# timspilak/cloud_merger

Hardware: AMD Instinct MI355X
Metric: merged+voxelized points/sec at 5 cm leaf, 4×1 M-pt inputs; HBM GB/s fraction (higher is better)
Workload: dtype f32

## Files before the change

### cloud_merger_amd/csrc/cm_common.hpp

```cpp
#pragma once
#include <hip/hip_runtime.h>
#include <stddef.h>
#include <stdint.h>

#include "cm_device.h"

namespace {

struct Pt { float x, y, z, i; };

#if defined(__HIP_DEVICE_COMPILE__)
#define CM_GLOBAL_AS __attribute__((address_space(1)))
#else
#define CM_GLOBAL_AS
#endif
typedef const CM_GLOBAL_AS unsigned char* cm_gptr;
typedef float cm_v4f __attribute__((ext_vector_type(4)));

__device__ __forceinline__ float load_f32_unaligned(cm_gptr p) {
    float f;
    __builtin_memcpy(&f, (const void*)p, 4);
    return f;
}

// ... 347 lines not shown
    if (!overflow && d[0] * d[1] * d[2] > 2147483647LL) overflow = true;
    if (overflow) { g.status = CM_DEV_OVERFLOW; return; }
    unsigned long long cells = 1;
#pragma unroll
    for (int a = 0; a < 3; ++a) {
        const int lo = static_cast<int>(floorf(__fmul_rn(g.min_p[a], inv[a])));
        const int hi = static_cast<int>(floorf(__fmul_rn(g.max_p[a], inv[a])));
        g.min_b[a] = lo; g.max_b[a] = hi; g.div_b[a] = hi - lo + 1;
        cells *= static_cast<unsigned long long>(hi - lo + 1);
    }
    if (cells > 0xFFFFFFFFull) { g.status = CM_DEV_OVERFLOW; return; }
    uint32_t bits = 1;
    while (bits < 32 && (cells - 1) >> bits) ++bits;
    g.key_bits = bits;
    g.n_passes = (bits + CM_RADIX_BITS - 1) / CM_RADIX_BITS;
}

struct BoxGrid {
    float inv0, inv1, inv2, fb0, fb1, fb2;
    uint32_t d0, d1, d2;
    uint32_t mul1, mul2l, mul2h;
};

__device__ __forceinline__ BoxGrid box_grid_of(const CmFrameDev* __restrict__ fd, int use_cell = 0) {
    BoxGrid b;
    const int32_t* min_b = use_cell ? fd->cell_min_b : fd->box_min_b;
    const int32_t* div_b = use_cell ? fd->cell_div_b : fd->box_div_b;
    const float* inv = use_cell ? fd->inv_cell : fd->inv_leaf;
    b.inv0 = inv[0]; b.inv1 = inv[1]; b.inv2 = inv[2];
    b.fb0 = static_cast<float>(min_b[0]); b.fb1 = static_cast<float>(min_b[1]); b.fb2 = static_cast<float>(min_b[2]);
    b.d0 = static_cast<uint32_t>(div_b[0]); b.d1 = static_cast<uint32_t>(div_b[1]); b.d2 = static_cast<uint32_t>(div_b[2]);
    b.mul1 = b.d0;
    const uint32_t mul2 = b.d0 * b.d1;
    b.mul2l = mul2 & 0xFFFu; b.mul2h = mul2 >> 12;
    return b;
}

__device__ __forceinline__ uint32_t box_index(const BoxGrid& b, uint32_t c0, uint32_t c1, uint32_t c2) {
    uint32_t hi = __umul24(c2, b.mul2h);
    asm("" : "+v"(hi));
    return c0 + __umul24(c1, b.mul1) + __umul24(c2, b.mul2l) + (hi << 12);
}

__device__ __forceinline__ uint32_t key_of(const BoxGrid& b, float x, float y, float z, bool* inside) {
    const uint32_t c0 = static_cast<uint32_t>(static_cast<int>(__fsub_rn(floorf(__fmul_rn(x, b.inv0)), b.fb0)));
    const uint32_t c1 = static_cast<uint32_t>(static_cast<int>(__fsub_rn(floorf(__fmul_rn(y, b.inv1)), b.fb1)));
    const uint32_t c2 = static_cast<uint32_t>(static_cast<int>(__fsub_rn(floorf(__fmul_rn(z, b.inv2)), b.fb2)));
// ... 237 lines not shown
```

### cloud_merger_amd/csrc/cm_kernels.h

```cpp
#pragma once
#include <hip/hip_runtime.h>
#include <stdint.h>

#include "cm_device.h"

void cmk_setup(hipStream_t s, const CmFrameDev& f, CmFrameDev* d_frame, CmTileDev* d_tiles);
void cmk_minmax(hipStream_t s, const CmFrameDev* fd, float* partials, uint32_t n_blocks, const unsigned char* mask);
void cmk_keys(hipStream_t s, const CmFrameDev* fd, CmFrameState* st, uint32_t* keys, uint32_t* hist,
              uint32_t* grp_acc, uint32_t* grp_clear_a, uint32_t* grp_clear_b, uint32_t n_group_words,
              uint32_t n_clear_a_words, uint32_t* seg_groups, uint32_t n_seg_groups, const float* partials,
              uint32_t n_partials, int from_crop, int use_cell, const unsigned char* mask,
              const CmFrameState* st_outlier, uint32_t n_tiles);
void cmk_outlier_mask(hipStream_t s, const CmFrameDev* fd, const CmFrameState* st, const uint32_t* keys_a,
                      const uint32_t* vals_a, const uint32_t* keys_b, const uint32_t* vals_b, void* sorted_pts,
                      void* rows, unsigned char* mask, uint32_t n_padded, const unsigned char* cls, uint32_t* pend_n,
                      bool already_gathered = false);
void cmk_sorted_rows(hipStream_t s, const CmFrameDev* fd, const CmFrameState* st, const uint32_t* keys_a, const uint32_t* vals_a,
                     const uint32_t* keys_b, const uint32_t* vals_b, void* sorted_pts, void* rows, uint32_t n_padded,
                     bool already_gathered);
void cmk_hist(hipStream_t s, const CmFrameState* st, const uint32_t* keys, uint32_t* hist, uint32_t* grp,
              uint32_t pass, uint32_t n_tiles);
void cmk_gscan(hipStream_t s, const CmFrameState* st, uint32_t* grp, uint32_t* totals, uint32_t pass,
               uint32_t n_groups);
void cmk_scatter(hipStream_t s, CmFrameState* st, const uint32_t* keys_in, const uint32_t* vals_in,
// ... 18 lines not shown
void cmk_merged(hipStream_t s, const CmFrameDev* fd, uint32_t* tile_counts, uint32_t* total, void* out,
                uint32_t n_tiles, const unsigned char* mask);

void cmk2_hist0(hipStream_t s, const CmFrameDev& f, CmFrameDev* fd, CmTileDev* tiles, bool do_setup, CmFrameState* st, uint32_t* hist, uint32_t* grp_acc,
                uint32_t* grp_clear_a, uint32_t* grp_clear_b, uint32_t n_group_words, uint32_t n_clear_a_words,
                unsigned long long* tile_state, uint32_t n_tile_state, float* records, int grid_mode, int check_box,
                uint32_t shift0, uint32_t n_global_passes, uint32_t n_tiles, const unsigned char* mask,
                const CmFrameState* st_outlier, int use_cell = 0, void* compact_out = nullptr, uint32_t* wave_cnt = nullptr);
void cmk2_hist(hipStream_t s, const CmFrameState* st, const unsigned char* dig, uint32_t* hist, uint32_t* grp,
               uint32_t n_tiles);
void cmk2_scatter(hipStream_t s, bool first, const CmFrameDev* fd, const CmTileDev* tiles, CmFrameState* st, const void* rec_in, void* rec_out,
                  unsigned char* dig_out, const uint32_t* hist, const uint32_t* grp, const uint32_t* totals,
                  uint32_t shift, uint32_t next_shift, uint32_t n_tiles, uint32_t n_groups, uint32_t n_padded,
                  const float* records, uint32_t n_records, int fold, const unsigned char* mask, int use_cell = 0,
                  const void* compact_in = nullptr, const uint32_t* wave_cnt = nullptr, int debug_swap = 0,
                  uint32_t* tile_kept = nullptr, bool sparse = false,
                  bool ballot = false);
void cmk2_local(hipStream_t s, const CmFrameDev* fd, CmFrameState* st, CmFrameState* st_next, uint32_t* host_state,
                const void* rec, unsigned long long* tile_state, uint32_t* ticket, void* out, uint32_t* out_key,
                uint32_t* out_cnt, void* partial_out, uint32_t low_bits, uint32_t n_padded);
void cmk2_local_sort(hipStream_t s, const CmFrameDev* fd, CmFrameState* st, uint32_t* host_state, const void* rec,
                     uint32_t* keys_sorted, void* recs_sorted, uint32_t low_bits, uint32_t n_padded);

void cmk3_local(hipStream_t s, const CmFrameDev* fd, CmFrameState* st, uint32_t* host_state, const void* rec, void* tile_info,
                uint32_t* grp_cnt, void* stage, uint32_t* stage_key, uint32_t* stage_cnt, bool partial, uint32_t low_bits,
                uint32_t n_slots,
                const uint32_t* spl = nullptr, const uint32_t* bofs = nullptr, uint32_t n_buckets = 0, uint32_t* spl_next = nullptr,
                bool ballot = false,
                uint32_t sub_shift = 0,
                const unsigned char* dig = nullptr);
void cmk3_local_big(hipStream_t s, const CmFrameDev* fd, CmFrameState* st, uint32_t* host_state, const void* rec, void* tile_info,
                    uint32_t* grp_cnt, void* stage, uint32_t* stage_key, uint32_t* stage_cnt, const uint32_t* spl, const uint32_t* bofs,
                    uint32_t n_buckets, uint32_t* spl_next, const uint32_t* big_list, bool ballot);
void cmk3_compact(hipStream_t s, const CmFrameState* st, CmFrameState* st_next, uint32_t* host_state, const void* tile_info,
                  const uint32_t* grp_cnt, const void* stage, const uint32_t* stage_key, const uint32_t* stage_cnt, void* out,
                  uint32_t* out_key, uint32_t* out_cnt, bool partial, uint32_t n_padded, uint32_t n_buckets = 0);

void cmk4_hist(hipStream_t s, const CmFrameDev& f, CmFrameDev* fd, CmTileDev* tiles, bool do_setup, CmFrameState* st,
               const uint32_t* spl, uint32_t* cnt, uint16_t* bid, unsigned long long* tile_state, uint32_t n_tile_state, float* records,
               int grid_mode, int check_box, uint32_t n_tiles,
               uint32_t n_buckets,
               uint32_t* big_list,
               uint32_t sub_shift,
               uint32_t* resident);
void cmk4_colscan(hipStream_t s, CmFrameState* st, uint32_t* host_state, uint32_t* cnt, uint32_t* totals, uint32_t n_tiles,
                  uint32_t cap, uint32_t cap_big, uint32_t* big_list);
void cmk4_scatter(hipStream_t s, const CmFrameDev* fd, const CmTileDev* tiles, CmFrameState* st, const uint16_t* bid,
                  const uint32_t* cnt, const uint32_t* totals, uint32_t* bofs, uint32_t n_buckets, void* rec_out,
                  const float* records, uint32_t n_records, int fold, uint32_t* tile_kept, uint32_t n_tiles,
                  unsigned char* dig_out,
                  bool ballot = false, const uint32_t* big_list = nullptr,
                  uint32_t sub_shift = 0);

void cmkg_setup(hipStream_t s, const CmGroundDev& g, CmGroundDev* d_ground);
// ... 59 lines not shown
```

### cloud_merger_amd/csrc/cm_kernels_v3.hip

```cpp
#include <hip/hip_runtime.h>
#include <stddef.h>
#include <stdint.h>

#include "cm_common.hpp"
#include "cm_device.h"
#include "cm_kernels.h"

namespace {

__device__ __forceinline__ float wave_sum_f32_fixed(float v) {
#define CM3_FADD(ctrl, rmask) v = __fadd_rn(v, __int_as_float(__builtin_amdgcn_update_dpp(0, __float_as_int(v), ctrl, rmask, 0xf, false)))
    CM3_FADD(0x111, 0xf); CM3_FADD(0x112, 0xf); CM3_FADD(0x114, 0xf); CM3_FADD(0x118, 0xf);
    CM3_FADD(0x142, 0xa); CM3_FADD(0x143, 0xc);
#undef CM3_FADD
    return __int_as_float(__builtin_amdgcn_readlane(__float_as_int(v), 63));
}

#define SCAL(x) static_cast<uint32_t>(__builtin_amdgcn_readfirstlane(static_cast<int>(x)))

struct Job3 {
    uint32_t p, key, kid, cnt;
    float sx, sy, sz, sw;
};
#define CM3_EXT_SEQ 16u
#define CM3_RUN_MAX (1u << 20)

CM_PHASE_DECLARE(g_phase_k3);

template <int LT, int LCAP, int LBLOCK, int WPS, bool PARTIAL, bool QUANT, bool BALLOT, bool SUB>
__global__ __launch_bounds__(LBLOCK, WPS) void k3_local(const CmFrameDev* __restrict__ fd,
                                                      CmFrameState* __restrict__ st,
                                                      uint32_t* __restrict__ host_state,
                                                      const float4* __restrict__ rec,
                                                      uint2* __restrict__ tile_info,
                                                      uint32_t* __restrict__ grp_cnt,
                                                      float4* __restrict__ stage,
                                                      uint32_t* __restrict__ stage_key,
                                                      uint32_t* __restrict__ stage_cnt,
                                                      uint32_t low_bits,
                                                      const uint32_t* __restrict__ spl, const uint32_t* __restrict__ bofs,
                                                      uint32_t n_buckets, uint32_t* __restrict__ spl_next,
                                                      const uint32_t* __restrict__ big_list, uint32_t sub_shift,
                                                      const unsigned char* __restrict__ dig) {
    constexpr int LWAVES = LBLOCK / 64, LITEMS = (LCAP + LBLOCK - 1) / LBLOCK, EXT0 = LBLOCK < 256 ? LBLOCK : 256;
    constexpr int WB = SUB ? 9 : 10, BINS = 1 << WB, HWORDS = BINS / 2;
    constexpr uint32_t MAXJ = LWAVES * HWORDS * 4 / sizeof(Job3);
    static_assert(LT == 4 * LBLOCK && LCAP <= 0x7FFE && HWORDS <= LBLOCK && LWAVES * HWORDS * 2 >= LCAP, "tile geometry");
    __shared__ uint32_t sk[LCAP];
    __shared__ uint16_t si[LCAP];
    __shared__ uint32_t whist[LWAVES][HWORDS];
    __shared__ uint32_t lds[2 * LWAVES];
    __shared__ uint32_t s_a, s_keyprev, s_bad, s_njobs;
    __shared__ uint16_t sp[SUB ? LCAP : 1];
    static_assert(!SUB || QUANT, "shared bins are a variant of the quantile finish");
    Job3* jobs = reinterpret_cast<Job3*>(&whist[0][0]);

    if (QUANT && big_list && blockIdx.x >= big_list[0]) return;
    PH_START();
    const int lane = threadIdx.x & 63;
    const uint32_t w = SCAL(threadIdx.x >> 6);
    if (st->status != CM_DEV_OK || st->outside) return;
    if (QUANT && st->quant_abort) return;
    const uint32_t n = SCAL(st->n_valid);
    const uint32_t n_lt = QUANT ? n_buckets : (n + LT - 1) / LT;
    uint32_t tile_ = blockIdx.x;
    if (SUB) {
        const uint32_t x = blockIdx.x & 7u, j = blockIdx.x >> 3;
        tile_ = (((((j >> sub_shift) << 3) + x) << sub_shift) + (j & ((1u << sub_shift) - 1u)));
    }
    if (QUANT && big_list) {
        if (tile_ >= SCAL(big_list[0])) return;
        tile_ = SCAL(big_list[1 + tile_]);
    }
    const uint32_t tile = tile_;
    if (tile >= n_lt) return;
    const BoxGrid b = box_grid_of(fd);
    const uint32_t L = QUANT ? 1u : low_bits;
    const uint32_t min_pts = SCAL((!PARTIAL && fd->min_pts > 1) ? fd->min_pts : 1u);

    const uint32_t bin = SUB ? tile >> sub_shift : tile;
    uint32_t base = QUANT ? SCAL(bofs[bin]) : tile * LT;
    const uint32_t rbase = base;
    const uint32_t q_end = QUANT ? SCAL(bofs[bin + 1]) : 0u;
    bool q_big = QUANT && !SUB && (q_end - base) > static_cast<uint32_t>(LCAP);
    if (QUANT && q_big && !big_list && (q_end - base) <= CM4_CAP_BIG) return;
    uint32_t nom = QUANT ? (q_big ? 0u : q_end - base) : min(static_cast<uint32_t>(LT), n - base);
    const uint32_t key_end = QUANT ? (fd->box_key_bits < 32u ? (1u << fd->box_key_bits) : 0xFFFFFFFFu) : 0u;
    const uint32_t q_lo = QUANT ? SCAL(spl[tile]) : 0u;
    const uint32_t q_hi = QUANT ? min(SCAL(spl[tile + 1]), key_end) : 0u;
    bool q_bad = false;
    if (SUB) {
        const uint32_t sub = tile & ((1u << sub_shift) - 1u);
        uint32_t kept = 0, below_t = 0;
        for (uint32_t off = rbase & ~15u; off < q_end; off += 16 * LBLOCK) {
            const uint32_t p0 = off + 16 * threadIdx.x;
            uint4 d = make_uint4(0xFFFFFFFFu, 0xFFFFFFFFu, 0xFFFFFFFFu, 0xFFFFFFFFu);
            if (p0 < q_end) d = *reinterpret_cast<const uint4*>(dig + p0);
            const uint32_t dw[4] = {d.x, d.y, d.z, d.w};
            uint32_t mm = 0;
#pragma unroll
            for (int i = 0; i < 16; ++i) {
                const uint32_t p = p0 + i, v = (dw[i >> 2] >> (8 * (i & 3))) & 0xFFu;
                const bool valid = p >= rbase && p < q_end;
                mm |= (valid && v == sub) ? (1u << i) : 0u;
                below_t += (valid && v < sub) ? 1u : 0u;
            }
            uint32_t tot;
            uint32_t pos = kept + block_excl_scan<LWAVES>(static_cast<uint32_t>(__builtin_popcount(mm)), lds, &tot);
            while (mm) {
                const uint32_t i = static_cast<uint32_t>(__builtin_ctz(mm));
                mm &= mm - 1u;
                if (pos < static_cast<uint32_t>(LCAP)) sp[pos] = static_cast<uint16_t>(p0 + i - rbase);
                ++pos;
            }
            kept += SCAL(tot);
        }
        uint32_t below;
        (void)block_excl_scan<LWAVES>(below_t, lds, &below);
        base = rbase + SCAL(below);
        q_big = kept > static_cast<uint32_t>(LCAP);
        nom = q_big ? 0u : kept;
        __syncthreads();
    }
    if (QUANT) {
        constexpr int HALF = LITEMS / 2;
#pragma unroll
        for (int h = 0; h < 2; ++h) {
            if (h == 1 && nom <= static_cast<uint32_t>(HALF * LBLOCK)) break;
            float4 r4[HALF];
#pragma unroll
            for (int r = 0; r < HALF; ++r) {
                const uint32_t q = (h * HALF + r) * LBLOCK + threadIdx.x;
                r4[r] = (q < nom) ? rec[rbase + (SUB ? sp[q < nom ? q : 0u] : q)] : make_float4(0.f, 0.f, 0.f, 0.f);
            }
#pragma unroll
            for (int r = 0; r < HALF; ++r) {
                const uint32_t q = (h * HALF + r) * LBLOCK + threadIdx.x;
                if (q < nom) {
                    const uint32_t k = key_of(b, r4[r]);
                    sk[q] = k;
                    q_bad = q_bad || k < q_lo || k >= q_hi;
                }
            }
        }
        if (threadIdx.x == 0) { s_keyprev = 0u; s_a = 0u; s_bad = 0u; s_njobs = 0u; }
    } else {
        float4 r4[4];
#pragma unroll
        for (int r = 0; r < 4; ++r) {
            const uint32_t q = r * LBLOCK + threadIdx.x;
            r4[r] = (q < nom) ? rec[base + q] : make_float4(0.f, 0.f, 0.f, 0.f);
        }
        const uint32_t j0 = base + LT + threadIdx.x;
        const bool has_e = threadIdx.x < EXT0 && nom == LT && j0 < n;
        const float4 e4 = has_e ? rec[j0] : make_float4(0.f, 0.f, 0.f, 0.f);
        float4 pv = make_float4(0.f, 0.f, 0.f, 0.f);
        if (threadIdx.x == 0 && base > 0) pv = rec[base - 1];
#pragma unroll
        for (int r = 0; r < 4; ++r) {
            const uint32_t q = r * LBLOCK + threadIdx.x;
            if (q < nom) sk[q] = key_of(b, r4[r]);
        }
        if (has_e) sk[LT + threadIdx.x] = key_of(b, e4);
        if (threadIdx.x == 0) { s_keyprev = base > 0 ? key_of(b, pv) : 0u; s_a = 0xFFFFFFFFu; s_bad = 0u; s_njobs = 0u; }
    }
    __syncthreads();
    PH(g_phase_k3, 0);

    bool bad_order = q_bad;
    if (!QUANT) {
        uint32_t best = 0xFFFFFFFFu;
#pragma unroll
        for (int r = 3; r >= 0; --r) {
            const uint32_t q = r * LBLOCK + threadIdx.x;
            if (q < nom) {
                const uint32_t kp = (q == 0) ? s_keyprev : sk[q - 1];
                const uint32_t hq = sk[q] >> L, hp = kp >> L;
                if ((base + q == 0) || (hq != hp)) best = q;
                bad_order = bad_order || (base + q > 0 && hq < hp);
            }
// ... 361 lines not shown
                    emit(jb.kid, jkey, tx, ty, tz, tw, tc);
                }
                __syncthreads();
            }
        }
    }
    PH(g_phase_k3, 5);
    if (threadIdx.x == 0) {
        tile_info[tile] = make_uint2(QUANT ? base : (a == 0xFFFFFFFFu ? 0u : a), c_t);
        if (c_t) atomicAdd(&grp_cnt[tile >> 6], c_t);
    }
}

template <int LT, bool PARTIAL>
__global__ __launch_bounds__(256) void k3_compact(const CmFrameState* __restrict__ st, CmFrameState* __restrict__ st_next,
                                                  uint32_t* __restrict__ host_state, const uint2* __restrict__ tile_info,
                                                  const uint32_t* __restrict__ grp_cnt, const float4* __restrict__ stage,
                                                  const uint32_t* __restrict__ stage_key, const uint32_t* __restrict__ stage_cnt,
                                                  float4* __restrict__ out, uint32_t* __restrict__ out_key,
                                                  uint32_t* __restrict__ out_cnt, uint32_t n_buckets) {
    __shared__ uint32_t lds[4];
    if (blockIdx.x == 0 && st_next && threadIdx.x < sizeof(CmFrameState) / 4)
        reinterpret_cast<uint32_t*>(st_next)[threadIdx.x] = 0;
    if (st->status != CM_DEV_OK || st->outside) {
        if (blockIdx.x == 0) report_state(host_state, st, st->status, 0u, true);
        return;
    }
    const uint32_t n = st->n_valid;
    if (n == 0) {
        if (blockIdx.x == 0) report_state(host_state, st, CM_DEV_EMPTY, 0u, true);
        return;
    }
    const uint32_t n_lt = n_buckets ? n_buckets : (n + LT - 1) / LT;
    const uint32_t tile = blockIdx.x;
    if (n_buckets && st->quant_abort) {
        if (blockIdx.x == 0) report_state(host_state, st, st->status, 0u, true);
        return;
    }
    if (tile == 0 && threadIdx.x == 0 && n_lt > gridDim.x) host_state[offsetof(CmFrameState, err) / 4] = CM_DEV_ERR_GRID;
    if (tile >= n_lt) return;
    const uint2 info = tile_info[tile];
    if (info.y == 0 && tile != n_lt - 1) return;
    const uint32_t g = tile >> 6;
    uint32_t s = 0;
    for (uint32_t q = threadIdx.x; q < g; q += 256) s += grp_cnt[q];
    for (uint32_t q = (g << 6) + threadIdx.x; q < tile; q += 256) s += tile_info[q].y;
    s = wave_sum_u32(s);
    if ((threadIdx.x & 63) == 0) lds[threadIdx.x >> 6] = s;
    __syncthreads();
    const uint32_t prefix = lds[0] + lds[1] + lds[2] + lds[3];
    if (tile == n_lt - 1) report_state(host_state, st, CM_DEV_OK, prefix + info.y, true);
    const size_t src = n_buckets ? static_cast<size_t>(info.x) : static_cast<size_t>(tile) * LT + info.x;
    for (uint32_t q = threadIdx.x; q < info.y; q += 256) {
        if (PARTIAL) {
            out[2 * (static_cast<size_t>(prefix) + q)] = stage[2 * (src + q)];
            out[2 * (static_cast<size_t>(prefix) + q) + 1] = stage[2 * (src + q) + 1];
        } else {
            const float4 sm = stage[src + q];
            const uint32_t cn = stage_cnt[src + q];
            const float c = static_cast<float>(cn);
            const float rc = __frcp_rn(c);
            out[prefix + q] = make_float4(centroid_div_rc(sm.x, c, rc), centroid_div_rc(sm.y, c, rc), centroid_div_rc(sm.z, c, rc),
                                          centroid_div_rc(sm.w, c, rc));
            if (out_key) { out_key[prefix + q] = stage_key[src + q]; out_cnt[prefix + q] = cn; }
        }
    }
}

}
#ifdef CM_PHASE_TIMING
extern "C" __attribute__((visibility("default"))) void cm_debug_phases3(unsigned long long* out, int reset) {
    phase_readout(HIP_SYMBOL(g_phase_k3), out, reset);
}
#endif

void cmk3_local(hipStream_t s, const CmFrameDev* fd, CmFrameState* st, uint32_t* host_state, const void* rec, void* tile_info,
                uint32_t* grp_cnt, void* stage, uint32_t* stage_key, uint32_t* stage_cnt, bool partial, uint32_t low_bits,
                uint32_t n_padded, const uint32_t* spl, const uint32_t* bofs, uint32_t n_buckets, uint32_t* spl_next, bool ballot,
                uint32_t sub_shift, const unsigned char* dig) {
    static_assert(CM4_CAP == 4032, "k4_colscan's capacity check is this kernel's LCAP");
    const dim3 grid(n_buckets ? (sub_shift ? ((((n_buckets + (1u << sub_shift) - 1u) >> sub_shift) + 7u) / 8u * 8u) << sub_shift : n_buckets)
                              : n_padded / 2048);
#define CM3_LOCAL_(PART, QUANT, BAL, SUB, SK, SC, SPL, BOFS, NB, NEXT)                                                              \
    hipLaunchKernelGGL((k3_local<2048, 4032, 512, 8, PART, QUANT, BAL, SUB>), grid, dim3(512), 0, s, fd, st, host_state,            \
                       reinterpret_cast<const float4*>(rec), reinterpret_cast<uint2*>(tile_info), grp_cnt,                          \
                       reinterpret_cast<float4*>(stage), SK, SC, low_bits, SPL, BOFS, NB, NEXT, nullptr, sub_shift, dig)
#define CM3_LOCAL(PART, QUANT, BAL, SK, SC, SPL, BOFS, NB, NEXT) CM3_LOCAL_(PART, QUANT, BAL, false, SK, SC, SPL, BOFS, NB, NEXT)
    if (n_buckets && sub_shift) { if (ballot) CM3_LOCAL_(false, true, true, true, stage_key, stage_cnt, spl, bofs, n_buckets, spl_next);
                                  else CM3_LOCAL_(false, true, false, true, stage_key, stage_cnt, spl, bofs, n_buckets, spl_next); }
    else if (n_buckets) { if (ballot) CM3_LOCAL(false, true, true, stage_key, stage_cnt, spl, bofs, n_buckets, spl_next);
                     else CM3_LOCAL(false, true, false, stage_key, stage_cnt, spl, bofs, n_buckets, spl_next); }
    else if (partial) { if (ballot) CM3_LOCAL(true, false, true, nullptr, nullptr, nullptr, nullptr, 0u, nullptr);
                        else CM3_LOCAL(true, false, false, nullptr, nullptr, nullptr, nullptr, 0u, nullptr); }
    else { if (ballot) CM3_LOCAL(false, false, true, stage_key, stage_cnt, nullptr, nullptr, 0u, spl_next);
           else CM3_LOCAL(false, false, false, stage_key, stage_cnt, nullptr, nullptr, 0u, spl_next); }
#undef CM3_LOCAL
#undef CM3_LOCAL_
}

void cmk3_local_big(hipStream_t s, const CmFrameDev* fd, CmFrameState* st, uint32_t* host_state, const void* rec, void* tile_info,
                    uint32_t* grp_cnt, void* stage, uint32_t* stage_key, uint32_t* stage_cnt, const uint32_t* spl, const uint32_t* bofs,
                    uint32_t n_buckets, uint32_t* spl_next, const uint32_t* big_list, bool ballot) {
#define CM3_BIG(BAL) hipLaunchKernelGGL((k3_local<4096, CM4_CAP_BIG, 1024, 4, false, true, BAL, false>), dim3(CM4_MAX_BIG), dim3(1024), 0, s, fd, st,   \
                                        host_state, reinterpret_cast<const float4*>(rec), reinterpret_cast<uint2*>(tile_info), grp_cnt,         \
                                        reinterpret_cast<float4*>(stage), stage_key, stage_cnt, 0u, spl, bofs, n_buckets, spl_next, big_list, 0u, nullptr)
    if (ballot) CM3_BIG(true); else CM3_BIG(false);
#undef CM3_BIG
}

void cmk3_compact(hipStream_t s, const CmFrameState* st, CmFrameState* st_next, uint32_t* host_state, const void* tile_info,
                  const uint32_t* grp_cnt, const void* stage, const uint32_t* stage_key, const uint32_t* stage_cnt, void* out,
                  uint32_t* out_key, uint32_t* out_cnt, bool partial, uint32_t n_padded, uint32_t n_buckets) {
    const dim3 grid(n_buckets ? n_buckets : n_padded / 2048);
    if (partial)
        hipLaunchKernelGGL((k3_compact<2048, true>), grid, dim3(256), 0, s, st, st_next, host_state,
                           reinterpret_cast<const uint2*>(tile_info), grp_cnt, reinterpret_cast<const float4*>(stage),
                           nullptr, nullptr, reinterpret_cast<float4*>(out), nullptr, nullptr, 0u);
    else
        hipLaunchKernelGGL((k3_compact<2048, false>), grid, dim3(256), 0, s, st, st_next, host_state,
                           reinterpret_cast<const uint2*>(tile_info), grp_cnt, reinterpret_cast<const float4*>(stage),
                           stage_key, stage_cnt, reinterpret_cast<float4*>(out), out_key, out_cnt, n_buckets);
}
```

### cloud_merger_amd/csrc/cm_kernels_v4.hip

```cpp
#include <hip/hip_runtime.h>
#include <stddef.h>
#include <stdint.h>

#include "cm_common.hpp"
#include "cm_device.h"
#include "cm_kernels.h"

namespace {

static_assert(CM4_BINS == 2048 && CM4_MAX_BUCKETS == 8192, "eleven to thirteen levels");
template <int LEVELS>
__device__ __forceinline__ void load_splitter_tree(uint32_t* __restrict__ tree, const uint32_t* __restrict__ spl_g) {
#pragma unroll
    for (int q = 0; q < (1 << LEVELS) / CM2_BLOCK; ++q) {
        const uint32_t e = q * CM2_BLOCK + threadIdx.x;
        const uint32_t l = 31u - static_cast<uint32_t>(__builtin_clz(e | 1u));
        const uint32_t p = e - (1u << l);
        tree[e] = e ? spl_g[((2u * p + 1u) << (LEVELS - 1 - l))] : 0u;
    }
}
template <int LEVELS, int N>
__device__ __forceinline__ void buckets_of(const uint32_t* __restrict__ tree, const uint32_t (&key)[N], uint32_t (&bk)[N]) {
#pragma unroll
    for (int r = 0; r < N; ++r) bk[r] = 4;
// ... 112 lines not shown
        uint32_t tx_ = threadIdx.x;
        asm volatile("" : "+v"(tx_));
#pragma unroll
        for (int q = 0; q < CM4_BINS / 2 / CM2_BLOCK; ++q) {
            cnt[cnt_at(tile, q * CM2_BLOCK + tx_, n_tiles)] = lh[q * CM2_BLOCK + tx_];
            lh[q * CM2_BLOCK + tx_] = 0;
        }
        if (predicted && tx_ < 8) records[static_cast<size_t>(tile) * 8 + tx_] = MinMax3::record_word<CM2_WAVES>(s_mm, s_cnt, tx_);
        PH_ACC(g_phase_k4, 5);
        PH_COUNT(g_phase_k4, 15);
        if (!more) break;
        __syncthreads();
        te = ten; tile = tile_n;
    }
    if (threadIdx.x == 0 && s_out) st->outside = 1u;
}

static_assert(32 * 128 >= CM4_MAX_TILES, "k4_colscan's register tile covers the frames the host sends here");
template <int CM4_SCAN_TPC>
__global__ __launch_bounds__(1024) void k4_colscan(CmFrameState* __restrict__ st, uint32_t* __restrict__ host_state,
                                                   uint32_t* __restrict__ cnt, uint32_t* __restrict__ totals,
                                                   uint32_t n_tiles, uint32_t cap, uint32_t cap_big, uint32_t* __restrict__ big_list) {
    __shared__ uint32_t s_lo[16][8], s_hi[16][8];
    if (st->status != CM_DEV_OK || st->outside) return;
    const uint32_t j = threadIdx.x & 7u, c = threadIdx.x >> 3;
    const uint32_t tpc = (n_tiles + 127u) / 128u;
    const uint32_t word = blockIdx.x * 8u + j;
    uint32_t v[CM4_SCAN_TPC];
    uint32_t lo = 0, hi = 0;
#pragma unroll
    for (int k = 0; k < CM4_SCAN_TPC; ++k) {
        const uint32_t t = c * tpc + k;
        v[k] = (static_cast<uint32_t>(k) < tpc && t < n_tiles) ? cnt[cnt_at(t, word, n_tiles)] : 0u;
        lo += v[k] & 0xFFFFu; hi += v[k] >> 16;
    }
    const int lane = threadIdx.x & 63, w = threadIdx.x >> 6;
    uint32_t ilo = lo, ihi = hi;
#pragma unroll
    for (int d = 8; d < 64; d <<= 1) {
        const uint32_t a = __shfl_up(ilo, d), b2 = __shfl_up(ihi, d);
        if (lane >= d) { ilo += a; ihi += b2; }
    }
    if (lane >= 56) { s_lo[w][j] = ilo; s_hi[w][j] = ihi; }
    __syncthreads();
    uint32_t plo = ilo - lo, phi = ihi - hi;
#pragma unroll
    for (int q = 0; q < 16; ++q) {
        const uint32_t a = s_lo[q][j], b2 = s_hi[q][j];
        if (q < w) { plo += a; phi += b2; }
    }
    uint32_t run = plo | (phi << 16);
#pragma unroll
    for (int k = 0; k < CM4_SCAN_TPC; ++k) {
        const uint32_t t = c * tpc + k;
        if (static_cast<uint32_t>(k) < tpc && t < n_tiles) cnt[cnt_at(t, word, n_tiles)] = run;
        run += v[k];
    }
    if (c == 127u) {
// ... 17 lines not shown
    }
}

template <bool SUB, bool BALLOT>
__global__ __launch_bounds__(CM2_BLOCK, 6) void k4_scatter(const CmFrameDev* __restrict__ fd, const CmTileDev* __restrict__ tiles,
                                                           CmFrameState* __restrict__ st, const uint16_t* __restrict__ bid,
                                                           const uint32_t* __restrict__ cnt, const uint32_t* __restrict__ totals,
                                                           uint32_t* __restrict__ bofs, uint32_t n_buckets,
                                                           float4* __restrict__ rec_out, const float* __restrict__ records,
                                                           uint32_t n_records, int fold, uint32_t* __restrict__ tile_kept,
                                                           unsigned char* __restrict__ dig_out, const uint32_t* __restrict__ big_list,
                                                           uint32_t sub_shift) {
    auto bin_of = [&](uint32_t id) { return SUB ? id >> sub_shift : id; };
    constexpr int HW = CM4_BINS / 2;
    constexpr int STG = 2048;
    __shared__ uint32_t buf[STG * 4 + STG / 2];
    __shared__ uint32_t gofs[CM4_BINS];
    __shared__ uint32_t lds[CM2_WAVES];
    static_assert(CM2_WAVES * HW <= STG * 4 + STG / 2 && CM4_BINS <= STG * 4, "overlays fit");
    static_assert(HW == 2 * CM2_BLOCK, "two counter words per thread");
    uint32_t (*wcnt)[HW] = reinterpret_cast<uint32_t (*)[HW]>(buf);
    float4* srec = reinterpret_cast<float4*>(buf);
    uint16_t* sbk = reinterpret_cast<uint16_t*>(buf + STG * 4);
    if (st->status != CM_DEV_OK) return;
    if (st->outside) {
        if (fold && blockIdx.x == 0) fold_bounds(reinterpret_cast<float*>(buf), st, records, n_records);
        return;
    }
    if (st->quant_abort) return;
    const uint32_t tile = xcd_tile(blockIdx.x, gridDim.x);
    const int lane = threadIdx.x & 63, w = threadIdx.x >> 6;

    const CmTileDev te = tiles[tile];
    const uint32_t sidx = static_cast<uint32_t>(__builtin_amdgcn_readfirstlane(static_cast<int>(te.info & 0xFFu)));
    Pt p[CM2_ITEMS];
    load_tile_te<CM2_ITEMS, true>(te, fd->s[sidx], w * (64 * CM2_ITEMS) + lane, p);
    uint32_t bk[CM2_ITEMS];
    {
        const uint32_t slot0 = tile * CM_TILE + w * (64 * CM2_ITEMS) + lane;
#pragma unroll
        for (int r = 0; r < CM2_ITEMS; ++r) bk[r] = bid[slot0 + r * 64];
    }
    for (uint32_t q = threadIdx.x; q < CM2_WAVES * HW; q += CM2_BLOCK) buf[q] = 0;

    float4 rec[CM2_ITEMS];
    uint32_t vmask = 0;
    {
        const CmSensorDev& sd = fd->s[sidx];
        float m[12];
        load_matrix(sd, m);
        const bool all_fields = fd->downsample_all != 0;
#pragma unroll
        for (int r = 0; r < CM2_ITEMS; ++r) {
            xf_point(m, p[r], rec[r].x, rec[r].y, rec[r].z);
            rec[r].w = all_fields ? p[r].i : 0.f;
            vmask |= (bk[r] != 0xFFFFu) ? (1u << r) : 0u;
            bk[r] &= SUB ? (CM4_MAX_BUCKETS - 1) : (CM4_BINS - 1);
        }
    }
    __syncthreads();
    const uint2 trow = *reinterpret_cast<const uint2*>(cnt + cnt_at(tile, 2 * threadIdx.x, gridDim.x));
    const uint4 tot4 = *reinterpret_cast<const uint4*>(totals + 4 * threadIdx.x);
    if (BALLOT) {
#pragma unroll
        for (int r = 0; r < CM2_ITEMS; ++r)
// ... 135 lines not shown
```

### cloud_merger_amd/csrc/cm_launch.cpp

```cpp
#include <algorithm>
#include <cmath>
#include <cstdio>
#include <cstring>
#include <limits>

#include "cm_ctx.hpp"

void prof_mark(cm_ctx* c, const char* name) {
    if (!(c->flags & CM_FLAG_PROFILE)) return;
    if (c->prof_used >= c->prof_ev.size()) {
        hipEvent_t e;
        if (hipEventCreate(&e) != hipSuccess) return;
        c->prof_ev.push_back(e);
        c->prof_names.emplace_back();
    }
    c->prof_names[c->prof_used] = name;
    (void)hipEventRecord(c->prof_ev[c->prof_used], c->stream);
    ++c->prof_used;
}

namespace {

bool descriptor_changed(cm_ctx* c) {
    if (c->frame_uploaded_valid && std::memcmp(&c->frame, &c->frame_uploaded, sizeof c->frame) == 0) return false;
// ... 110 lines not shown
    CmFrameState* state = c->d_state[c->cur];
    CmFrameState* state_next = c->d_state[c->cur ^ 1];
    c->from_crop = pl.b_grid_mode == 1 || (pl.b_grid_mode == 2 && !pl.predicted);
    c->frame_mask = mask;
    const uint32_t nt = f.n_tiles;
    const bool ballot = !c->route.lds_rank;
    uint32_t* skey = c->out_key ? c->keys_a : nullptr;
    if (pl.quant) {
        const uint32_t nb = pl.nb, sub = pl.sub;
        const uint32_t nbins = (nb + (1u << sub) - 1u) >> sub;
        const uint32_t* spl = c->spl[c->route.spl_cur];
        uint32_t* spl_next = c->spl[c->route.spl_cur ^ 1];
        prof_mark(c, "k4_hist");
        cmk4_hist(st, f, c->d_frame, c->d_tiles, do_setup, state, spl, c->qcnt, c->qbid, c->tile_state, pl.n_tile_state, c->records,
                  pl.b_grid_mode, pl.predicted ? 1 : 0, nt, nb, sub ? nullptr : c->qbig, sub, c->hist_resident);
        prof_mark(c, "k4_colscan");
        if (sub) cmk4_colscan(st, state, c->h_state_dev, c->qcnt, c->qtot, nt, CM4_CAP << sub, CM4_CAP << sub, nullptr);
        else cmk4_colscan(st, state, c->h_state_dev, c->qcnt, c->qtot, nt, CM4_CAP, pl.big_armed ? CM4_CAP_BIG : CM4_CAP, c->qbig);
        prof_mark(c, "k4_scatter");
        cmk4_scatter(st, c->d_frame, c->d_tiles, state, c->qbid, c->qcnt, c->qtot, c->qbofs, nbins, c->rec_a, c->records, nt,
                     pl.predicted ? 1 : 0, c->d_tile_kept, nt, sub ? c->dig : nullptr, ballot, sub ? nullptr : c->qbig, sub);
        uint32_t* grp_cnt = reinterpret_cast<uint32_t*>(c->tile_state + nb);
        prof_mark(c, "k3_local");
        cmk3_local(st, c->d_frame, state, c->h_state_dev, c->rec_a, c->tile_state, grp_cnt, c->rec_b, skey, c->vals_a, false, 0u,
                   0u, spl, c->qbofs, nb, spl_next, ballot, sub, sub ? c->dig : nullptr);
        if (pl.big_armed) {
            prof_mark(c, "k3_local(big)");
            cmk3_local_big(st, c->d_frame, state, c->h_state_dev, c->rec_a, c->tile_state, grp_cnt, c->rec_b, skey, c->vals_a, spl,
                           c->qbofs, nb, spl_next, c->qbig, ballot);
        }
        prof_mark(c, "k3_compact");
        cmk3_compact(st, state, state_next, c->h_state_dev, c->tile_state, grp_cnt, c->rec_b, skey, c->vals_a, c->out, c->out_key,
                     c->out_cnt, false, 0u, nb);
        return end_frame(c);
    }
    if (pl.mode == 1 && !c->partial) HIP_TRY(c, hipMalloc(&c->partial, static_cast<size_t>(c->cap_padded) * 32));
    const GrpArrays g = next_grp(c);
    prof_mark(c, "k2_hist0");
    cmk2_hist0(st, f, c->d_frame, c->d_tiles, do_setup, state, c->hist, g.p0, g.p0_next, g.rest, g.gw, g.stride, c->tile_state,
               f.n_padded / 1024 + 2, c->records, pl.b_grid_mode, pl.predicted ? 1 : 0, pl.low, pl.g, nt, mask, st_outlier, 0,
               pl.pack ? c->rec_b : nullptr, c->wave_cnt);
    record_passes(c, state, g, pl.g, pl.low, pl.nt_later, mask, 0, pl.predicted ? 1 : 0, pl.pack, pl.sparse,
                  c->route.debug_misrank != 0, ballot, c->d_tile_kept, "k2_scatter");
    const void* rec_sorted = ((pl.g - 1) & 1u) ? c->rec_b : c->rec_a;
    if (pl.k3) {
        void* stage = ((pl.g - 1) & 1u) ? c->rec_a : c->rec_b;
        if (pl.mode == 1) {
            if (!c->stage32) HIP_TRY(c, hipMalloc(&c->stage32, static_cast<size_t>(c->cap_padded) * 32));
            stage = c->stage32;
        }
        uint32_t* grp_cnt = reinterpret_cast<uint32_t*>(c->tile_state + f.n_padded / 2048);
        prof_mark(c, "k3_local");
        uint32_t* spl_next = pl.mode == 0 ? c->spl[c->route.spl_cur ^ 1] : nullptr;
        cmk3_local(st, c->d_frame, state, c->h_state_dev, rec_sorted, c->tile_state, grp_cnt, stage, skey, c->vals_a, pl.mode == 1,
                   pl.low, pl.nt_later * CM_TILE, nullptr, nullptr, 0u, spl_next, ballot);
        prof_mark(c, "k3_compact");
        cmk3_compact(st, state, state_next, c->h_state_dev, c->tile_state, grp_cnt, stage, skey, c->vals_a,
                     pl.mode == 1 ? c->partial : c->out, c->out_key, c->out_cnt, pl.mode == 1, pl.nt_later * CM_TILE);
    } else {
        prof_mark(c, "k2_local");
        cmk2_local(st, c->d_frame, state, state_next, c->h_state_dev, rec_sorted, c->tile_state,
                   reinterpret_cast<uint32_t*>(c->tile_state + (f.n_padded / 1024 + 1)), c->out, c->out_key, c->out_cnt,
                   pl.mode == 1 ? c->partial : nullptr, pl.low, f.n_padded);
    }
    return end_frame(c);
}

void keys_and_sort(cm_ctx* c, CmFrameState* stg, int gmode, int use_cell, const unsigned char* mask,
                   const CmFrameState* st_outlier, uint32_t n_pass) {
    const CmFrameDev& f = c->frame;
    const uint32_t nt = f.n_tiles;
    const uint32_t n_seg_groups = (f.n_padded / CM_SEG_TILE + CM_SEG_GROUP - 1) / CM_SEG_GROUP + 1;
    const uint32_t n_partials = nt < CM_MINMAX_BLOCKS ? nt : CM_MINMAX_BLOCKS;
    const GrpArrays g = next_grp(c);
    prof_mark(c, use_cell ? "k_keys(outlier)" : "k_keys");
    cmk_keys(c->stream, c->d_frame, stg, c->keys_a, c->hist, g.p0, g.p0_next, g.rest, g.gw, g.stride, c->seg_groups, n_seg_groups,
             c->partials, n_partials, gmode, use_cell, mask, st_outlier, nt);
// ... 660 lines not shown
```

Measured before the change: 42.86 billion.

## Pass frame grid by value and issue status/bucket loads before early-exit checks

k3_local now takes a host-computed K3Frame (box grid, min_pts, key bits) as a kernel argument instead of dereferencing the device frame struct. In k3_local, k3_compact, k4_colscan and k4_scatter, the status flags, bucket offsets, splitters, prefix-sum operands and tile descriptor are all loaded up front and pinned to scalar registers before the early-return checks. This puts the dependent global loads in flight together and removes serial load-then-branch latency at kernel start. Phase-timing markers are also added. The cost is some speculative loads on blocks that then exit, plus the assumption that the host copy of the frame matches the device copy.

```diff
diff --git a/cloud_merger_amd/csrc/cm_common.hpp b/cloud_merger_amd/csrc/cm_common.hpp
--- a/cloud_merger_amd/csrc/cm_common.hpp
+++ b/cloud_merger_amd/csrc/cm_common.hpp
@@ -393,7 +393,7 @@
     uint32_t mul1, mul2l, mul2h;
 };
 
-__device__ __forceinline__ BoxGrid box_grid_of(const CmFrameDev* __restrict__ fd, int use_cell = 0) {
+__host__ __device__ __forceinline__ BoxGrid box_grid_of(const CmFrameDev* __restrict__ fd, int use_cell = 0) {
     BoxGrid b;
     const int32_t* min_b = use_cell ? fd->cell_min_b : fd->box_min_b;
     const int32_t* div_b = use_cell ? fd->cell_div_b : fd->box_div_b;
diff --git a/cloud_merger_amd/csrc/cm_kernels.h b/cloud_merger_amd/csrc/cm_kernels.h
--- a/cloud_merger_amd/csrc/cm_kernels.h
+++ b/cloud_merger_amd/csrc/cm_kernels.h
@@ -64,14 +64,14 @@
 void cmk2_local_sort(hipStream_t s, const CmFrameDev* fd, CmFrameState* st, uint32_t* host_state, const void* rec,
                      uint32_t* keys_sorted, void* recs_sorted, uint32_t low_bits, uint32_t n_padded);
 
-void cmk3_local(hipStream_t s, const CmFrameDev* fd, CmFrameState* st, uint32_t* host_state, const void* rec, void* tile_info,
+void cmk3_local(hipStream_t s, const CmFrameDev& f, CmFrameState* st, uint32_t* host_state, const void* rec, void* tile_info,
                 uint32_t* grp_cnt, void* stage, uint32_t* stage_key, uint32_t* stage_cnt, bool partial, uint32_t low_bits,
                 uint32_t n_slots,
                 const uint32_t* spl = nullptr, const uint32_t* bofs = nullptr, uint32_t n_buckets = 0, uint32_t* spl_next = nullptr,
                 bool ballot = false,
                 uint32_t sub_shift = 0,
                 const unsigned char* dig = nullptr);
-void cmk3_local_big(hipStream_t s, const CmFrameDev* fd, CmFrameState* st, uint32_t* host_state, const void* rec, void* tile_info,
+void cmk3_local_big(hipStream_t s, const CmFrameDev& f, CmFrameState* st, uint32_t* host_state, const void* rec, void* tile_info,
                     uint32_t* grp_cnt, void* stage, uint32_t* stage_key, uint32_t* stage_cnt, const uint32_t* spl, const uint32_t* bofs,
                     uint32_t n_buckets, uint32_t* spl_next, const uint32_t* big_list, bool ballot);
 void cmk3_compact(hipStream_t s, const CmFrameState* st, CmFrameState* st_next, uint32_t* host_state, const void* tile_info,
diff --git a/cloud_merger_amd/csrc/cm_kernels_v3.hip b/cloud_merger_amd/csrc/cm_kernels_v3.hip
--- a/cloud_merger_amd/csrc/cm_kernels_v3.hip
+++ b/cloud_merger_amd/csrc/cm_kernels_v3.hip
@@ -27,8 +27,20 @@
 
 CM_PHASE_DECLARE(g_phase_k3);
 
+struct K3Frame {
+    BoxGrid b;
+    uint32_t min_pts, box_key_bits;
+};
+K3Frame k3_frame_of(const CmFrameDev& f) {
+    K3Frame kf;
+    kf.b = box_grid_of(&f);
+    kf.min_pts = f.min_pts;
+    kf.box_key_bits = f.box_key_bits;
+    return kf;
+}
+
 template <int LT, int LCAP, int LBLOCK, int WPS, bool PARTIAL, bool QUANT, bool BALLOT, bool SUB>
-__global__ __launch_bounds__(LBLOCK, WPS) void k3_local(const CmFrameDev* __restrict__ fd,
+__global__ __launch_bounds__(LBLOCK, WPS) void k3_local(const K3Frame kf,
                                                       CmFrameState* __restrict__ st,
                                                       uint32_t* __restrict__ host_state,
                                                       const float4* __restrict__ rec,
@@ -55,39 +67,52 @@
     static_assert(!SUB || QUANT, "shared bins are a variant of the quantile finish");
     Job3* jobs = reinterpret_cast<Job3*>(&whist[0][0]);
 
-    if (QUANT && big_list && blockIdx.x >= big_list[0]) return;
     PH_START();
+    PH_MARK(th_);
     const int lane = threadIdx.x & 63;
     const uint32_t w = SCAL(threadIdx.x >> 6);
-    if (st->status != CM_DEV_OK || st->outside) return;
-    if (QUANT && st->quant_abort) return;
-    const uint32_t n = SCAL(st->n_valid);
-    const uint32_t n_lt = QUANT ? n_buckets : (n + LT - 1) / LT;
     uint32_t tile_ = blockIdx.x;
     if (SUB) {
         const uint32_t x = blockIdx.x & 7u, j = blockIdx.x >> 3;
         tile_ = (((((j >> sub_shift) << 3) + x) << sub_shift) + (j & ((1u << sub_shift) - 1u)));
     }
-    if (QUANT && big_list) {
-        if (tile_ >= SCAL(big_list[0])) return;
-        tile_ = SCAL(big_list[1 + tile_]);
-    }
-    const uint32_t tile = tile_;
-    if (tile >= n_lt) return;
-    const BoxGrid b = box_grid_of(fd);
+    uint32_t s_status = static_cast<uint32_t>(st->status), s_outside = st->outside, s_abort = QUANT ? st->quant_abort : 0u, s_n = st->n_valid;
+    uint32_t h_big_n = 0, h_big_b = 0, h_b0 = 0, h_b1 = 0, h_s0 = 0, h_s1 = 0;
+    if (QUANT) {
+        if (big_list) {
+            h_big_n = big_list[0];
+            h_big_b = big_list[1 + blockIdx.x];
+        } else {
+            const uint32_t tc = min(tile_, static_cast<uint32_t>(CM4_MAX_BUCKETS - 1)), bc = min(SUB ? tc >> sub_shift : tc, static_cast<uint32_t>(CM4_BINS - 1));
+            h_b0 = bofs[bc]; h_b1 = bofs[bc + 1];
+            h_s0 = spl[tc]; h_s1 = spl[tc + 1];
+        }
+    }
+    asm volatile("" : "+s"(s_status), "+s"(s_outside), "+s"(s_abort), "+s"(s_n), "+s"(h_big_n), "+s"(h_big_b), "+s"(h_b0), "+s"(h_b1),
+                      "+s"(h_s0), "+s"(h_s1));
+    const uint32_t n = s_n;
+    const uint32_t n_lt = QUANT ? n_buckets : (n + LT - 1) / LT;
+    const bool big = QUANT && big_list;
+    const uint32_t tile = big ? h_big_b : tile_;
+    if (s_status != CM_DEV_OK || s_outside || s_abort || (big && blockIdx.x >= h_big_n) || tile >= n_lt) return;
+    if (threadIdx.x == 0) PH_SINCE(g_phase_k3, 6, th_);
+    if (big) {
+        h_b0 = SCAL(bofs[tile]); h_b1 = SCAL(bofs[tile + 1]);
+        h_s0 = SCAL(spl[tile]); h_s1 = SCAL(spl[tile + 1]);
+    }
+    const BoxGrid b = kf.b;
     const uint32_t L = QUANT ? 1u : low_bits;
-    const uint32_t min_pts = SCAL((!PARTIAL && fd->min_pts > 1) ? fd->min_pts : 1u);
-
-    const uint32_t bin = SUB ? tile >> sub_shift : tile;
-    uint32_t base = QUANT ? SCAL(bofs[bin]) : tile * LT;
+    const uint32_t min_pts = (!PARTIAL && kf.min_pts > 1) ? kf.min_pts : 1u;
+
+    uint32_t base = QUANT ? h_b0 : tile * LT;
     const uint32_t rbase = base;
-    const uint32_t q_end = QUANT ? SCAL(bofs[bin + 1]) : 0u;
+    const uint32_t q_end = QUANT ? h_b1 : 0u;
     bool q_big = QUANT && !SUB && (q_end - base) > static_cast<uint32_t>(LCAP);
     if (QUANT && q_big && !big_list && (q_end - base) <= CM4_CAP_BIG) return;
     uint32_t nom = QUANT ? (q_big ? 0u : q_end - base) : min(static_cast<uint32_t>(LT), n - base);
-    const uint32_t key_end = QUANT ? (fd->box_key_bits < 32u ? (1u << fd->box_key_bits) : 0xFFFFFFFFu) : 0u;
-    const uint32_t q_lo = QUANT ? SCAL(spl[tile]) : 0u;
-    const uint32_t q_hi = QUANT ? min(SCAL(spl[tile + 1]), key_end) : 0u;
+    const uint32_t key_end = QUANT ? (kf.box_key_bits < 32u ? (1u << kf.box_key_bits) : 0xFFFFFFFFu) : 0u;
+    const uint32_t q_lo = QUANT ? h_s0 : 0u;
+    const uint32_t q_hi = QUANT ? min(h_s1, key_end) : 0u;
     bool q_bad = false;
     if (SUB) {
         const uint32_t sub = tile & ((1u << sub_shift) - 1u);
@@ -133,6 +158,7 @@
                 const uint32_t q = (h * HALF + r) * LBLOCK + threadIdx.x;
                 r4[r] = (q < nom) ? rec[rbase + (SUB ? sp[q < nom ? q : 0u] : q)] : make_float4(0.f, 0.f, 0.f, 0.f);
             }
+            if (h == 0) { PH_LOADS_BACK(); if (threadIdx.x == 0) PH_SINCE(g_phase_k3, 7, th_); }
 #pragma unroll
             for (int r = 0; r < HALF; ++r) {
                 const uint32_t q = (h * HALF + r) * LBLOCK + threadIdx.x;
@@ -156,6 +182,8 @@
         const float4 e4 = has_e ? rec[j0] : make_float4(0.f, 0.f, 0.f, 0.f);
         float4 pv = make_float4(0.f, 0.f, 0.f, 0.f);
         if (threadIdx.x == 0 && base > 0) pv = rec[base - 1];
+        PH_LOADS_BACK();
+        if (threadIdx.x == 0) PH_SINCE(g_phase_k3, 7, th_);
 #pragma unroll
         for (int r = 0; r < 4; ++r) {
             const uint32_t q = r * LBLOCK + threadIdx.x;
@@ -563,29 +591,29 @@
     __shared__ uint32_t lds[4];
     if (blockIdx.x == 0 && st_next && threadIdx.x < sizeof(CmFrameState) / 4)
         reinterpret_cast<uint32_t*>(st_next)[threadIdx.x] = 0;
-    if (st->status != CM_DEV_OK || st->outside) {
-        if (blockIdx.x == 0) report_state(host_state, st, st->status, 0u, true);
-        return;
-    }
-    const uint32_t n = st->n_valid;
-    if (n == 0) {
-        if (blockIdx.x == 0) report_state(host_state, st, CM_DEV_EMPTY, 0u, true);
-        return;
-    }
+    PH_MARK(th_);
+    const uint32_t tile = blockIdx.x, g = tile >> 6;
+    uint32_t s_status = static_cast<uint32_t>(st->status), s_outside = st->outside, s_n = st->n_valid, s_abort = st->quant_abort;
+    uint2 info = tile_info[tile];
+    const uint32_t q0 = threadIdx.x, q1 = (g << 6) + threadIdx.x;
+    const uint32_t w0 = grp_cnt[q0 < g ? q0 : (g ? g - 1u : 0u)];
+    const uint32_t w1 = tile_info[q1 < tile ? q1 : tile].y;
+    uint32_t s = (q0 < g ? w0 : 0u) + (q1 < tile ? w1 : 0u);
+    for (uint32_t q = q0 + 256; q < g; q += 256) s += grp_cnt[q];
+    for (uint32_t q = q1 + 256; q < tile; q += 256) s += tile_info[q].y;
+    asm volatile("" : "+s"(s_status), "+s"(s_outside), "+s"(s_n), "+s"(s_abort), "+s"(info.x), "+s"(info.y), "+v"(s));
+    const uint32_t n = s_n;
     const uint32_t n_lt = n_buckets ? n_buckets : (n + LT - 1) / LT;
-    const uint32_t tile = blockIdx.x;
-    if (n_buckets && st->quant_abort) {
-        if (blockIdx.x == 0) report_state(host_state, st, st->status, 0u, true);
+    const bool not_ok = s_status != CM_DEV_OK || s_outside;
+    const bool aborted = n_buckets && s_abort;
+    if (not_ok || n == 0 || aborted) {
+        if (blockIdx.x == 0) report_state(host_state, st, (!not_ok && n == 0) ? CM_DEV_EMPTY : static_cast<int>(s_status), 0u, true);
         return;
     }
     if (tile == 0 && threadIdx.x == 0 && n_lt > gridDim.x) host_state[offsetof(CmFrameState, err) / 4] = CM_DEV_ERR_GRID;
     if (tile >= n_lt) return;
-    const uint2 info = tile_info[tile];
     if (info.y == 0 && tile != n_lt - 1) return;
-    const uint32_t g = tile >> 6;
-    uint32_t s = 0;
-    for (uint32_t q = threadIdx.x; q < g; q += 256) s += grp_cnt[q];
-    for (uint32_t q = (g << 6) + threadIdx.x; q < tile; q += 256) s += tile_info[q].y;
+    if (threadIdx.x == 0) PH_SINCE(g_phase_k3, 8, th_);
     s = wave_sum_u32(s);
     if ((threadIdx.x & 63) == 0) lds[threadIdx.x >> 6] = s;
     __syncthreads();
@@ -599,6 +627,7 @@
         } else {
             const float4 sm = stage[src + q];
             const uint32_t cn = stage_cnt[src + q];
+            if (q == threadIdx.x) { PH_LOADS_BACK(); if (threadIdx.x == 0) PH_SINCE(g_phase_k3, 9, th_); }
             const float c = static_cast<float>(cn);
             const float rc = __frcp_rn(c);
             out[prefix + q] = make_float4(centroid_div_rc(sm.x, c, rc), centroid_div_rc(sm.y, c, rc), centroid_div_rc(sm.z, c, rc),
@@ -615,15 +644,16 @@
 }
 #endif
 
-void cmk3_local(hipStream_t s, const CmFrameDev* fd, CmFrameState* st, uint32_t* host_state, const void* rec, void* tile_info,
+void cmk3_local(hipStream_t s, const CmFrameDev& f, CmFrameState* st, uint32_t* host_state, const void* rec, void* tile_info,
                 uint32_t* grp_cnt, void* stage, uint32_t* stage_key, uint32_t* stage_cnt, bool partial, uint32_t low_bits,
                 uint32_t n_padded, const uint32_t* spl, const uint32_t* bofs, uint32_t n_buckets, uint32_t* spl_next, bool ballot,
                 uint32_t sub_shift, const unsigned char* dig) {
     static_assert(CM4_CAP == 4032, "k4_colscan's capacity check is this kernel's LCAP");
+    const K3Frame kf = k3_frame_of(f);
     const dim3 grid(n_buckets ? (sub_shift ? ((((n_buckets + (1u << sub_shift) - 1u) >> sub_shift) + 7u) / 8u * 8u) << sub_shift : n_buckets)
                               : n_padded / 2048);
 #define CM3_LOCAL_(PART, QUANT, BAL, SUB, SK, SC, SPL, BOFS, NB, NEXT)                                                              \
-    hipLaunchKernelGGL((k3_local<2048, 4032, 512, 8, PART, QUANT, BAL, SUB>), grid, dim3(512), 0, s, fd, st, host_state,            \
+    hipLaunchKernelGGL((k3_local<2048, 4032, 512, 8, PART, QUANT, BAL, SUB>), grid, dim3(512), 0, s, kf, st, host_state,            \
                        reinterpret_cast<const float4*>(rec), reinterpret_cast<uint2*>(tile_info), grp_cnt,                          \
                        reinterpret_cast<float4*>(stage), SK, SC, low_bits, SPL, BOFS, NB, NEXT, nullptr, sub_shift, dig)
 #define CM3_LOCAL(PART, QUANT, BAL, SK, SC, SPL, BOFS, NB, NEXT) CM3_LOCAL_(PART, QUANT, BAL, false, SK, SC, SPL, BOFS, NB, NEXT)
@@ -639,10 +669,11 @@
 #undef CM3_LOCAL_
 }
 
-void cmk3_local_big(hipStream_t s, const CmFrameDev* fd, CmFrameState* st, uint32_t* host_state, const void* rec, void* tile_info,
+void cmk3_local_big(hipStream_t s, const CmFrameDev& f, CmFrameState* st, uint32_t* host_state, const void* rec, void* tile_info,
                     uint32_t* grp_cnt, void* stage, uint32_t* stage_key, uint32_t* stage_cnt, const uint32_t* spl, const uint32_t* bofs,
                     uint32_t n_buckets, uint32_t* spl_next, const uint32_t* big_list, bool ballot) {
-#define CM3_BIG(BAL) hipLaunchKernelGGL((k3_local<4096, CM4_CAP_BIG, 1024, 4, false, true, BAL, false>), dim3(CM4_MAX_BIG), dim3(1024), 0, s, fd, st,   \
+    const K3Frame kf = k3_frame_of(f);
+#define CM3_BIG(BAL) hipLaunchKernelGGL((k3_local<4096, CM4_CAP_BIG, 1024, 4, false, true, BAL, false>), dim3(CM4_MAX_BIG), dim3(1024), 0, s, kf, st,   \
                                         host_state, reinterpret_cast<const float4*>(rec), reinterpret_cast<uint2*>(tile_info), grp_cnt,         \
                                         reinterpret_cast<float4*>(stage), stage_key, stage_cnt, 0u, spl, bofs, n_buckets, spl_next, big_list, 0u, nullptr)
     if (ballot) CM3_BIG(true); else CM3_BIG(false);
diff --git a/cloud_merger_amd/csrc/cm_kernels_v4.hip b/cloud_merger_amd/csrc/cm_kernels_v4.hip
--- a/cloud_merger_amd/csrc/cm_kernels_v4.hip
+++ b/cloud_merger_amd/csrc/cm_kernels_v4.hip
@@ -158,7 +158,7 @@
                                                    uint32_t* __restrict__ cnt, uint32_t* __restrict__ totals,
                                                    uint32_t n_tiles, uint32_t cap, uint32_t cap_big, uint32_t* __restrict__ big_list) {
     __shared__ uint32_t s_lo[16][8], s_hi[16][8];
-    if (st->status != CM_DEV_OK || st->outside) return;
+    uint32_t s_status = static_cast<uint32_t>(st->status), s_outside = st->outside;
     const uint32_t j = threadIdx.x & 7u, c = threadIdx.x >> 3;
     const uint32_t tpc = (n_tiles + 127u) / 128u;
     const uint32_t word = blockIdx.x * 8u + j;
@@ -170,6 +170,8 @@
         v[k] = (static_cast<uint32_t>(k) < tpc && t < n_tiles) ? cnt[cnt_at(t, word, n_tiles)] : 0u;
         lo += v[k] & 0xFFFFu; hi += v[k] >> 16;
     }
+    asm volatile("" : "+s"(s_status), "+s"(s_outside), "+v"(lo), "+v"(hi));
+    if (s_status != CM_DEV_OK || s_outside) return;
     const int lane = threadIdx.x & 63, w = threadIdx.x >> 6;
     uint32_t ilo = lo, ihi = hi;
 #pragma unroll
@@ -233,25 +235,32 @@
     uint32_t (*wcnt)[HW] = reinterpret_cast<uint32_t (*)[HW]>(buf);
     float4* srec = reinterpret_cast<float4*>(buf);
     uint16_t* sbk = reinterpret_cast<uint16_t*>(buf + STG * 4);
-    if (st->status != CM_DEV_OK) return;
-    if (st->outside) {
-        if (fold && blockIdx.x == 0) fold_bounds(reinterpret_cast<float*>(buf), st, records, n_records);
-        return;
-    }
-    if (st->quant_abort) return;
+    PH_MARK(th_);
     const uint32_t tile = xcd_tile(blockIdx.x, gridDim.x);
     const int lane = threadIdx.x & 63, w = threadIdx.x >> 6;
-
-    const CmTileDev te = tiles[tile];
-    const uint32_t sidx = static_cast<uint32_t>(__builtin_amdgcn_readfirstlane(static_cast<int>(te.info & 0xFFu)));
-    Pt p[CM2_ITEMS];
-    load_tile_te<CM2_ITEMS, true>(te, fd->s[sidx], w * (64 * CM2_ITEMS) + lane, p);
+    uint32_t s_status = static_cast<uint32_t>(st->status), s_outside = st->outside, s_abort = st->quant_abort;
+    const CmTileDev te_ = tiles[tile];
+    unsigned long long te_data = reinterpret_cast<unsigned long long>(te_.data);
+    uint32_t te_n = te_.n_left, te_info = te_.info;
+    asm volatile("" : "+s"(s_status), "+s"(s_outside), "+s"(s_abort), "+s"(te_data), "+s"(te_n), "+s"(te_info));
+    if (s_status != CM_DEV_OK || s_outside || s_abort) {
+        if (s_status == CM_DEV_OK && s_outside && fold && blockIdx.x == 0) fold_bounds(reinterpret_cast<float*>(buf), st, records, n_records);
+        return;
+    }
+    if (threadIdx.x == 0) PH_SINCE(g_phase_k4, 8, th_);
+    CmTileDev te;
+    te.data = reinterpret_cast<const unsigned char*>(te_data); te.n_left = te_n; te.info = te_info;
+    const uint32_t sidx = te.info & 0xFFu;
     uint32_t bk[CM2_ITEMS];
     {
         const uint32_t slot0 = tile * CM_TILE + w * (64 * CM2_ITEMS) + lane;
 #pragma unroll
         for (int r = 0; r < CM2_ITEMS; ++r) bk[r] = bid[slot0 + r * 64];
     }
+    Pt p[CM2_ITEMS];
+    load_tile_te<CM2_ITEMS, true>(te, fd->s[sidx], w * (64 * CM2_ITEMS) + lane, p);
+    PH_LOADS_BACK();
+    if (threadIdx.x == 0) PH_SINCE(g_phase_k4, 9, th_);
     for (uint32_t q = threadIdx.x; q < CM2_WAVES * HW; q += CM2_BLOCK) buf[q] = 0;
 
     float4 rec[CM2_ITEMS];
diff --git a/cloud_merger_amd/csrc/cm_launch.cpp b/cloud_merger_amd/csrc/cm_launch.cpp
--- a/cloud_merger_amd/csrc/cm_launch.cpp
+++ b/cloud_merger_amd/csrc/cm_launch.cpp
@@ -156,11 +156,11 @@
                      pl.predicted ? 1 : 0, c->d_tile_kept, nt, sub ? c->dig : nullptr, ballot, sub ? nullptr : c->qbig, sub);
         uint32_t* grp_cnt = reinterpret_cast<uint32_t*>(c->tile_state + nb);
         prof_mark(c, "k3_local");
-        cmk3_local(st, c->d_frame, state, c->h_state_dev, c->rec_a, c->tile_state, grp_cnt, c->rec_b, skey, c->vals_a, false, 0u,
+        cmk3_local(st, f, state, c->h_state_dev, c->rec_a, c->tile_state, grp_cnt, c->rec_b, skey, c->vals_a, false, 0u,
                    0u, spl, c->qbofs, nb, spl_next, ballot, sub, sub ? c->dig : nullptr);
         if (pl.big_armed) {
             prof_mark(c, "k3_local(big)");
-            cmk3_local_big(st, c->d_frame, state, c->h_state_dev, c->rec_a, c->tile_state, grp_cnt, c->rec_b, skey, c->vals_a, spl,
+            cmk3_local_big(st, f, state, c->h_state_dev, c->rec_a, c->tile_state, grp_cnt, c->rec_b, skey, c->vals_a, spl,
                            c->qbofs, nb, spl_next, c->qbig, ballot);
         }
         prof_mark(c, "k3_compact");
@@ -186,7 +186,7 @@
         uint32_t* grp_cnt = reinterpret_cast<uint32_t*>(c->tile_state + f.n_padded / 2048);
         prof_mark(c, "k3_local");
         uint32_t* spl_next = pl.mode == 0 ? c->spl[c->route.spl_cur ^ 1] : nullptr;
-        cmk3_local(st, c->d_frame, state, c->h_state_dev, rec_sorted, c->tile_state, grp_cnt, stage, skey, c->vals_a, pl.mode == 1,
+        cmk3_local(st, f, state, c->h_state_dev, rec_sorted, c->tile_state, grp_cnt, stage, skey, c->vals_a, pl.mode == 1,
                    pl.low, pl.nt_later * CM_TILE, nullptr, nullptr, 0u, spl_next, ballot);
         prof_mark(c, "k3_compact");
         cmk3_compact(st, state, state_next, c->h_state_dev, c->tile_state, grp_cnt, stage, skey, c->vals_a,
```

Result: no change. 43.30 billion, median of 6 (+1.0%).
